# stwerner97/model-based-pde-control

Measured on AMD Instinct MI355X. Metric: KS sub-steps/sec (batched env), higher is better.
Workload: dtype f64

## Files before the change

model-based-pde-control_amd/csrc/fno.hip:

```cpp
#include <hip/hip_runtime.h>

#include <cstdio>
#include <map>
#include <mutex>
#include <utility>

#include "../../include/spectral/forward_select.h"
#include "../../include/spectral_hip.h"
#include "capi_error.h"

namespace {

typedef float f32x4 __attribute__((ext_vector_type(4)));

constexpr int C = 32;
constexpr int M = 16;
constexpr int K2 = 2 * M;
constexpr int KP = K2 + 4;
constexpr int KS = 2;
constexpr int TPB = 512;
constexpr int LAYERS = 4;

struct Weights {
    const float* lift_w;
    const float* lift_b;
    const float* wr[LAYERS];
    const float* wi[LAYERS];
    const float* pw[LAYERS];
    const float* pb[LAYERS];
    const float* p1_w;
    const float* p1_b;
    const float* p2_w;
    const float* p2_b;
};

struct Rows {
    const float* ptr;
    long stride_t, stride_b;
    __device__ const float* row(int t, int b) const { return ptr + t * stride_t + b * stride_b; }
};

struct FwdArgs {
    Weights w;
    Rows u, act;
    float* delta;
    float* out;
    float* pre;
    float* xspec;
    const float* tabg;
    int n, nb, pairs;
    int spec_pairs, spec_pair0;
    float cscale, cshift;
};

struct BwdArgs {
    Weights w;
    Rows u, act;
    const float* gdelta;
    const float* gout;
    int gout_t;
    const float* pre;
    float* gspec;
    float* rows;
    float* dbase;
    float* dact;
    const float* tabg;
    int n, nb, pairs;
    int spec_pairs, spec_pair0;
    float cscale;
};

constexpr int R_LIFT_W = 0, R_LIFT_B = 64, R_LAYER = 96, R_LAYER_SZ = 1024 + 32;
constexpr int R_P1W = R_LAYER + LAYERS * R_LAYER_SZ, R_P1B = R_P1W + 1024, R_P2W = R_P1B + 32, R_P2B = R_P2W + 32;
constexpr int ROW = ((R_P2B + 1 + 63) / 64) * 64;

__device__ __forceinline__ void gelu_parts(float x, float& cdf, float& pdf) {
    const float ax = fabsf(x);
    const float e = __expf(-0.5f * x * x);
    const float t = __frcp_rn(fmaf(0.3275911f * 0.70710678118654752f, ax, 1.0f));
    float poly = fmaf(1.061405429f, t, -1.453152027f);
    poly = fmaf(poly, t, 1.421413741f);
    poly = fmaf(poly, t, -0.284496736f);
    poly = fmaf(poly, t, 0.254829592f);
    const float erf_abs = fmaf(-poly * t, e, 1.0f);
    cdf = 0.5f * (1.0f + copysignf(erf_abs, x));
    pdf = 0.3989422804014327f * e;
}
__device__ __forceinline__ float gelu(float x) {
    float cdf, pdf;
    gelu_parts(x, cdf, pdf);
    return x * cdf;
}
__device__ __forceinline__ float gelu_grad(float x) {
    float cdf, pdf;
    gelu_parts(x, cdf, pdf);
    return fmaf(x, pdf, cdf);
}

#ifdef FNO_STAMP
__device__ unsigned long long g_stamps[256];
#define STAMP(k)                                                                      \
    do {                                                                              \
        if (blockIdx.x == 0 && threadIdx.x == 0) g_stamps[(k)] = __builtin_amdgcn_s_memtime(); \
    } while (0)
#else
#define STAMP(k) do { } while (0)
#endif

struct Lds {
    float *xs, *tb, *S, *Z, *wps, *gv, *misc;
    int NP;
    __device__ Lds(float* base, int N) {
        NP = N + 4;
        xs = base;
        tb = xs + C * NP;
        S = tb + C * NP;
        Z = S + KS * C * KP;
        wps = Z + C * KP;
        gv = wps + C * KP;
        misc = gv + N;
    }
    static size_t floats(int N) { return 2 * (size_t)C * (N + 4) + (KS + 2) * C * KP + (size_t)N + 256; }
};

__global__ void twiddle_init_kernel(float* tab, int N) {
    const int i = blockIdx.x * blockDim.x + threadIdx.x;
    if (i >= K2 * N) return;
    const int k = i / N, n = i - k * N;
    const bool is_sin = k >= M;
    const int mode = is_sin ? k - M : k;
    const int idx = (int)(((long)mode * n) % N);
    const float ang = 2.0f * (float)idx / (float)N;
    tab[i] = is_sin ? -sinpif(ang) : cospif(ang);
}
__device__ __forceinline__ void load_table(float* tab, const float* __restrict__ tabg, int N, int NP) {
    const int sh = __ffs(N) - 1;
    for (int i = threadIdx.x; i < (K2 * N) >> 2; i += blockDim.x) {
        const int e = i << 2, k = e >> sh, n = e & (N - 1);
        *reinterpret_cast<float4*>(tab + k * NP + n) = reinterpret_cast<const float4*>(tabg)[i];
    }
}

__device__ __forceinline__ void contract_n(const float* arows, const float* brows, float* S, int N, int NP) {
    const int lane = threadIdx.x & 63, wave = threadIdx.x >> 6, nwaves = blockDim.x >> 6;
    const int r = lane & 15, q = lane >> 4;
    for (int t = wave; t < 4 * KS; t += nwaves) {
        const int tile = t & 3, ks = t >> 2, rt = tile >> 1, ct = tile & 1;
        const int span = N / KS, kbeg = ks * span;
        const float* arow = arows + (16 * rt + r) * NP + kbeg;
        const float* brow = brows + (16 * ct + r) * NP + kbeg;
        f32x4 acc0 = {0.f, 0.f, 0.f, 0.f}, acc1 = {0.f, 0.f, 0.f, 0.f}, acc2 = {0.f, 0.f, 0.f, 0.f}, acc3 = {0.f, 0.f, 0.f, 0.f};
        for (int k0 = 0; k0 < span; k0 += 16) {
            const float a0 = arow[k0 + q], a1 = arow[k0 + 4 + q], a2 = arow[k0 + 8 + q], a3 = arow[k0 + 12 + q];
            const float b0 = brow[k0 + q], b1 = brow[k0 + 4 + q], b2 = brow[k0 + 8 + q], b3 = brow[k0 + 12 + q];
            acc0 = __builtin_amdgcn_mfma_f32_16x16x4f32(a0, b0, acc0, 0, 0, 0);
            acc1 = __builtin_amdgcn_mfma_f32_16x16x4f32(a1, b1, acc1, 0, 0, 0);
            acc2 = __builtin_amdgcn_mfma_f32_16x16x4f32(a2, b2, acc2, 0, 0, 0);
            acc3 = __builtin_amdgcn_mfma_f32_16x16x4f32(a3, b3, acc3, 0, 0, 0);
        }
        float* dst = S + ks * C * KP;
// ... 273 lines not shown
            const float* wrow = L.wps + (16 * rt + r) * KP;
#pragma unroll
            for (int k0 = 0; k0 < C; k0 += 4)
                acc = __builtin_amdgcn_mfma_f32_16x16x4f32(wrow[k0 + q], L.xs[(k0 + q) * NP + pos], acc, 0, 0, 0);
#pragma unroll
            for (int j = 0; j < 4; ++j) {
                const int row = 16 * rt + 4 * q + j;
                part = fmaf(L.misc[C + row], gelu(acc[j] + L.misc[row]), part);
            }
        }
        part += __shfl_xor(part, 16, 64);
        part += __shfl_xor(part, 32, 64);
        if (q == 0) {
            const float d = part + b2;
            out[pos] = fmaf(cscale, d, u[pos]) + cshift;
        }
    }
}

__device__ __forceinline__ float row_dot(const float* buf, const float* v, int N, int NP) {
    const int row = threadIdx.x >> 4, l16 = threadIdx.x & 15;
    float s = 0.0f;
    if (row < C) {
        const float* src = buf + row * NP;
        if (v) {
            for (int n = l16; n < N; n += 16) s = fmaf(src[n], v[n], s);
        } else {
            for (int n = l16; n < N; n += 16) s += src[n];
        }
    }
    s += __shfl_xor(s, 1, 64);
    s += __shfl_xor(s, 2, 64);
    s += __shfl_xor(s, 4, 64);
    s += __shfl_xor(s, 8, 64);
    return s;
}

__global__ void __launch_bounds__(TPB) fno_backward_kernel(const BwdArgs a) {
    extern __shared__ __align__(16) float lds_raw[];
    const int N = a.n;
    const Lds L(lds_raw, N);
    const int NP = L.NP;
    float* db = L.tb;
    const int p = blockIdx.x, t = p / a.nb, b = p - t * a.nb;
    const int lane = threadIdx.x & 63, wave = threadIdx.x >> 6, nwaves = blockDim.x >> 6;
    const int r = lane & 15, q = lane >> 4;
    const int sh = __ffs(N) - 1;
    const float* u = a.u.row(t, b);
    const float* act = a.act.row(t, b);
    float* grow = a.rows + (size_t)p * ROW;
    const float* pre_p = a.pre + (size_t)p * LAYERS * C * N;
    const bool has_gout = a.gout && t == a.gout_t;

    for (int n = threadIdx.x; n < N; n += blockDim.x) {
        float g = a.gdelta[(size_t)p * N + n];
        if (has_gout) g = fmaf(a.cscale, a.gout[(size_t)b * N + n], g);
        L.gv[n] = g;
    }
    {
        const float4* src = reinterpret_cast<const float4*>(pre_p + (size_t)(LAYERS - 1) * C * N);
        for (int i = threadIdx.x; i < (C * N) >> 2; i += blockDim.x) {
            const int e = i << 2, c = e >> sh, n = e & (N - 1);
            *reinterpret_cast<float4*>(L.xs + c * NP + n) = src[i];
        }
    }
    load_mat(L.wps, a.w.p1_w);
    if (threadIdx.x < C) {
        L.misc[threadIdx.x] = a.w.p1_b[threadIdx.x];
        L.misc[C + threadIdx.x] = a.w.p2_w[threadIdx.x];
    }
    __syncthreads();

    {
        float dw2[2][4] = {{0.f, 0.f, 0.f, 0.f}, {0.f, 0.f, 0.f, 0.f}};
        for (int ct = wave; ct < (N >> 4); ct += nwaves) {
            const int pos = 16 * ct + r;
            const float g = L.gv[pos];
#pragma unroll
            for (int rt = 0; rt < 2; ++rt) {
                f32x4 acc = {0.f, 0.f, 0.f, 0.f};
                const float* wrow = L.wps + (16 * rt + r) * KP;
#pragma unroll
                for (int k0 = 0; k0 < C; k0 += 4)
                    acc = __builtin_amdgcn_mfma_f32_16x16x4f32(wrow[k0 + q], L.xs[(k0 + q) * NP + pos], acc, 0, 0, 0);
#pragma unroll
                for (int j = 0; j < 4; ++j) {
                    const int row = 16 * rt + 4 * q + j;
                    const float z1 = acc[j] + L.misc[row];
                    dw2[rt][j] = fmaf(g, gelu(z1), dw2[rt][j]);
                    db[row * NP + pos] = L.misc[C + row] * g * gelu_grad(z1);
                }
            }
        }
#pragma unroll
        for (int rt = 0; rt < 2; ++rt)
#pragma unroll
            for (int j = 0; j < 4; ++j) {
                float v = dw2[rt][j];
                v += __shfl_xor(v, 1, 64);
                v += __shfl_xor(v, 2, 64);
                v += __shfl_xor(v, 4, 64);
                v += __shfl_xor(v, 8, 64);
                if (r == 0) L.Z[wave * C + 16 * rt + 4 * q + j] = v;
            }
    }
    __syncthreads();
    contract_n(db, L.xs, L.S, N, NP);
    {
        const float s = row_dot(db, nullptr, N, NP);
        if ((threadIdx.x & 15) == 0 && (threadIdx.x >> 4) < C) grow[R_P1B + (threadIdx.x >> 4)] = s;
        if (threadIdx.x < C) {
            float v = L.Z[threadIdx.x];
            for (int w = 1; w < TPB / 64; ++w) v += L.Z[w * C + threadIdx.x];
            grow[R_P2W + threadIdx.x] = v;
        }
        if (wave == 0) {
            float g = 0.0f;
            for (int n = lane; n < N; n += 64) g += L.gv[n];
#pragma unroll
            for (int m = 1; m < 64; m <<= 1) g += __shfl_xor(g, m, 64);
            if (lane == 0) grow[R_P2B] = g;
        }
    }
    __syncthreads();
    for (int i = threadIdx.x; i < C * C; i += blockDim.x) grow[R_P1W + i] = s_sum(L.S, (i >> 5) * KP + (i & 31));
    for (int ct = wave; ct < (N >> 4); ct += nwaves) {
        const int pos = 16 * ct + r;
        f32x4 acc[2];
#pragma unroll
        for (int rt = 0; rt < 2; ++rt) {
            acc[rt] = f32x4{0.f, 0.f, 0.f, 0.f};
#pragma unroll
            for (int k0 = 0; k0 < C; k0 += 4)
                acc[rt] = __builtin_amdgcn_mfma_f32_16x16x4f32(L.wps[(k0 + q) * KP + 16 * rt + r], db[(k0 + q) * NP + pos], acc[rt], 0, 0, 0);
        }
#pragma unroll
        for (int rt = 0; rt < 2; ++rt)
#pragma unroll
            for (int j = 0; j < 4; ++j) db[(16 * rt + 4 * q + j) * NP + pos] = acc[rt][j];
    }
    __syncthreads();

    const float s0 = 1.0f / (float)N, s1 = 2.0f / (float)N;
    for (int l = LAYERS - 1; l >= 0; --l) {
        if (l + 1 < LAYERS) {
            const float4* src = reinterpret_cast<const float4*>(pre_p + (size_t)l * C * N);
            for (int i = threadIdx.x; i < (C * N) >> 2; i += blockDim.x) {
                const int e = i << 2, c = e >> sh, n = e & (N - 1);
                const float4 v = src[i];
                float4* d = reinterpret_cast<float4*>(db + c * NP + n);
                float4 g = *d;
                g.x *= gelu_grad(v.x);
                g.y *= gelu_grad(v.y);
                g.z *= gelu_grad(v.z);
                g.w *= gelu_grad(v.w);
                *d = g;
            }
        }
        if (l > 0) {
            const float4* src = reinterpret_cast<const float4*>(pre_p + (size_t)(l - 1) * C * N);
            for (int i = threadIdx.x; i < (C * N) >> 2; i += blockDim.x) {
                const int e = i << 2, c = e >> sh, n = e & (N - 1);
                float4 v = src[i];
                v.x = gelu(v.x);
                v.y = gelu(v.y);
                v.z = gelu(v.z);
                v.w = gelu(v.w);
                *reinterpret_cast<float4*>(L.xs + c * NP + n) = v;
            }
        } else {
            lift_into(L.xs, u, act, a.w, N, NP);
        }
        load_mat(L.wps, a.w.pw[l]);
        __syncthreads();
        contract_n(db, L.xs, L.S, N, NP);
        {
            const float s = row_dot(db, nullptr, N, NP);
            if ((threadIdx.x & 15) == 0 && (threadIdx.x >> 4) < C) grow[R_LAYER + l * R_LAYER_SZ + 1024 + (threadIdx.x >> 4)] = s;
        }
        __syncthreads();
        for (int i = threadIdx.x; i < C * C; i += blockDim.x)
            grow[R_LAYER + l * R_LAYER_SZ + i] = s_sum(L.S, (i >> 5) * KP + (i & 31));
        load_table(L.xs, a.tabg, N, NP);
        __syncthreads();
        MixRegs mw;
        mix_load<true>(a.w.wr[l], a.w.wi[l], mw);
        contract_n(db, L.xs, L.S, N, NP);
        __syncthreads();
        for (int i = threadIdx.x; i < C * K2; i += blockDim.x) {
            const int k = i >> 5, c = i & 31, m = k & (M - 1);
            const float g = s_sum(L.S, c * KP + k) * (m == 0 ? s0 : s1);
            L.Z[c * KP + k] = g;
            a.gspec[(((size_t)l * K2 + k) * a.spec_pairs + a.spec_pair0 + p) * C + c] = g;
        }
        __syncthreads();
        mix_compute<true>(mw, L.Z, L.S, 1.0f, 1.0f);
        __syncthreads();
        for (int ct = wave; ct < (N >> 4); ct += nwaves) {
            const int pos = 16 * ct + r;
            f32x4 acc[2][2];
#pragma unroll
            for (int rt = 0; rt < 2; ++rt) {
                acc[rt][0] = f32x4{0.f, 0.f, 0.f, 0.f};
                acc[rt][1] = f32x4{0.f, 0.f, 0.f, 0.f};
                const float* zrow = L.S + (16 * rt + r) * KP;
#pragma unroll
                for (int k0 = 0; k0 < K2; k0 += 4) {
                    acc[rt][0] = __builtin_amdgcn_mfma_f32_16x16x4f32(zrow[k0 + q], L.xs[(k0 + q) * NP + pos], acc[rt][0], 0, 0, 0);
                    acc[rt][1] = __builtin_amdgcn_mfma_f32_16x16x4f32(L.wps[(k0 + q) * KP + 16 * rt + r], db[(k0 + q) * NP + pos], acc[rt][1], 0, 0, 0);
                }
            }
#pragma unroll
            for (int rt = 0; rt < 2; ++rt)
#pragma unroll
                for (int j = 0; j < 4; ++j) db[(16 * rt + 4 * q + j) * NP + pos] = acc[rt][0][j] + acc[rt][1][j];
        }
        __syncthreads();
    }

    for (int n = threadIdx.x; n < N; n += blockDim.x) {
        L.gv[n] = u[n];
        L.Z[n] = act[n];
    }
    if (threadIdx.x < C) {
        L.misc[threadIdx.x] = a.w.lift_w[2 * threadIdx.x];
        L.misc[C + threadIdx.x] = a.w.lift_w[2 * threadIdx.x + 1];
    }
    __syncthreads();
    {
        const float su = row_dot(db, L.gv, N, NP), sa = row_dot(db, L.Z, N, NP), sb = row_dot(db, nullptr, N, NP);
        if ((threadIdx.x & 15) == 0 && (threadIdx.x >> 4) < C) {
            const int c = threadIdx.x >> 4;
            grow[R_LIFT_W + 2 * c] = su;
            grow[R_LIFT_W + 2 * c + 1] = sa;
            grow[R_LIFT_B + c] = sb;
        }
    }
    if (a.dbase) {
        for (int n = threadIdx.x; n < N; n += blockDim.x) {
            float s = 0.0f;
#pragma unroll 8
            for (int c = 0; c < C; ++c) s = fmaf(L.misc[c], db[c * NP + n], s);
            if (has_gout) s += a.gout[(size_t)b * N + n];
            a.dbase[(size_t)p * N + n] = s;
        }
    }
    if (a.dact) {
        for (int n = threadIdx.x; n < N; n += blockDim.x) {
            float s = 0.0f;
#pragma unroll 8
            for (int c = 0; c < C; ++c) s = fmaf(L.misc[C + c], db[c * NP + n], s);
            a.dact[(size_t)p * N + n] = s;
        }
    }
}

__global__ void __launch_bounds__(512) fno_reduce_rows_kernel(const float* rows, int pairs, int width, float* out) {
    __shared__ float part[8][64];
    const int col = threadIdx.x & 63, grp = threadIdx.x >> 6;
    const int j = blockIdx.x * 64 + col;
    float s0 = 0.0f, s1 = 0.0f, s2 = 0.0f, s3 = 0.0f;
    if (j < width) {
        int p = grp;
        for (; p + 24 < pairs; p += 32) {
            s0 += rows[(size_t)p * width + j];
            s1 += rows[(size_t)(p + 8) * width + j];
            s2 += rows[(size_t)(p + 16) * width + j];
            s3 += rows[(size_t)(p + 24) * width + j];
        }
        for (; p < pairs; p += 8) s0 += rows[(size_t)p * width + j];
    }
    part[grp][col] = (s0 + s1) + (s2 + s3);
    __syncthreads();
    if (grp == 0 && j < width) {
        float v = part[0][col];
#pragma unroll
        for (int g = 1; g < 8; ++g) v += part[g][col];
        out[j] = v;
    }
}

struct WgradOut {
    float* dwr[LAYERS];
    float* dwi[LAYERS];
};

constexpr int WG_KS = 4;
__global__ void __launch_bounds__(256 * WG_KS) fno_spec_wgrad_kernel(const float* xspec, const float* gspec, int pairs, const WgradOut dst) {
    __shared__ float part[WG_KS][4][2][256];
    const int l = blockIdx.x / M, m = blockIdx.x % M;
    const int lane = threadIdx.x & 63, wave = threadIdx.x >> 6;
    const int tile = wave & 3, ks = wave >> 2;
    const int r = lane & 15, q = lane >> 4;
    const int rt = tile >> 1, ct = tile & 1;
    const size_t plane = (size_t)pairs * C;
    const float* xr = xspec + ((size_t)l * K2 + m) * plane;
    const float* xi = xspec + ((size_t)l * K2 + M + m) * plane;
    const float* gr = gspec + ((size_t)l * K2 + m) * plane;
    const float* gi = gspec + ((size_t)l * K2 + M + m) * plane;
    f32x4 rr = {0.f, 0.f, 0.f, 0.f}, ii = {0.f, 0.f, 0.f, 0.f}, ir = {0.f, 0.f, 0.f, 0.f}, ri = {0.f, 0.f, 0.f, 0.f};
    for (int p0 = 4 * ks; p0 < pairs; p0 += 4 * WG_KS) {
        const int pp = p0 + q;
        const bool ok = pp < pairs;
        const size_t row = (size_t)(ok ? pp : 0) * C;
        const float axr = ok ? xr[row + 16 * rt + r] : 0.f, axi = ok ? xi[row + 16 * rt + r] : 0.f;
        const float bgr = ok ? gr[row + 16 * ct + r] : 0.f, bgi = ok ? gi[row + 16 * ct + r] : 0.f;
// ... 150 lines not shown
    if (int rc = check(who, n, nb, nb, width, modes, layers)) return rc;
    SelectArgs k = {};
    for (int m = 0; m < a->members; ++m) {
        k.w[m] = weights_of(&a->w[m]);
        k.cscale[m] = a->cscale[m];
        k.cshift[m] = a->cshift[m];
    }
    k.chosen = a->chosen;
    k.step = a->step;
    k.u = a->u;
    k.act = a->act;
    k.out = a->out;
    k.members = a->members;
    k.T = a->T;
    k.n = n;
    k.nb = nb;
    int trc = 0;
    k.tabg = twiddle_table(who, n, (hipStream_t)stream, &trc);
    if (!k.tabg) return trc;
    return launch(fno_forward_select_kernel, who, stream, nb, n, k);
}

int fno_backward(void* stream, const fno_weights* w, int width, int modes, int layers, int n, int nb, int pairs, const float* u,
                 long u_stride_t, long u_stride_b, const float* act, long a_stride_t, long a_stride_b, float cscale,
                 const float* gdelta, const float* gout, int gout_t, const float* pre, float* gspec, int spec_pairs, int spec_pair0,
                 float* rows, float* dbase, float* dact) {
    if (!complete(w) || !u || !act || !gdelta || !pre || !gspec || !rows) return fail(-1, "fno_backward: bad argument");
    if (spec_pair0 < 0 || spec_pair0 + pairs > spec_pairs) return fail(-1, "fno_backward: spectra window out of range");
    if (int rc = check("fno_backward", n, nb, pairs, width, modes, layers)) return rc;
    BwdArgs a;
    a.w = weights_of(w);
    a.u = Rows{u, u_stride_t, u_stride_b};
    a.act = Rows{act, a_stride_t, a_stride_b};
    a.gdelta = gdelta;
    a.gout = gout;
    a.gout_t = gout_t;
    a.pre = pre;
    a.gspec = gspec;
    a.spec_pairs = spec_pairs;
    a.spec_pair0 = spec_pair0;
    a.rows = rows;
    a.dbase = dbase;
    a.dact = dact;
    int trc = 0;
    a.tabg = twiddle_table("fno_backward", n, (hipStream_t)stream, &trc);
    if (!a.tabg) return trc;
    a.n = n;
    a.nb = nb;
    a.pairs = pairs;
    a.cscale = cscale;
    return launch(fno_backward_kernel, "fno_backward", stream, pairs, n, a);
}

int fno_reduce_rows(void* stream, const float* rows, int pairs, float* out) {
    if (!rows || !out || pairs <= 0) return fail(-1, "fno_reduce_rows: bad argument");
    hipLaunchKernelGGL(fno_reduce_rows_kernel, dim3((ROW + 63) / 64), dim3(512), 0, (hipStream_t)stream, rows, pairs, ROW, out);
    return launch_status(-2, "fno_reduce_rows");
}

int fno_spec_wgrad(void* stream, const float* xspec, const float* gspec, int pairs, float* const* dwr, float* const* dwi) {
    if (!xspec || !gspec || !dwr || !dwi || pairs <= 0) return fail(-1, "fno_spec_wgrad: bad argument");
    WgradOut dst;
    for (int l = 0; l < LAYERS; ++l) {
        if (!dwr[l] || !dwi[l]) return fail(-1, "fno_spec_wgrad: NULL output");
        dst.dwr[l] = dwr[l];
        dst.dwi[l] = dwi[l];
    }
    hipLaunchKernelGGL(fno_spec_wgrad_kernel, dim3(LAYERS * M), dim3(256 * WG_KS), 0, (hipStream_t)stream, xspec, gspec, pairs, dst);
    return launch_status(-2, "fno_spec_wgrad");
}

const char* fno_last_error(void) { return g_err; }

#ifdef FNO_STAMP
int fno_read_stamps(unsigned long long* host, int n) {
    return hipMemcpyFromSymbol(host, HIP_SYMBOL(g_stamps), sizeof(unsigned long long) * (n < 256 ? n : 256)) == hipSuccess ? 0 : -2;
}
#endif

}
```

model-based-pde-control_amd/pdecontrol/surrogates/fno_hip.py:

```python
import ctypes

import torch

import hipbind
from pdecontrol.surrogates import spectral

_p, _i, _l, _f = ctypes.c_void_p, ctypes.c_int, ctypes.c_long, ctypes.c_float
WIDTH, MODES, LAYERS = 32, 16, 4


class FnoWeights(ctypes.Structure):
    _fields_ = [("lift_w", _p), ("lift_b", _p), ("spec_wr", _p * 4), ("spec_wi", _p * 4), ("pw_w", _p * 4), ("pw_b", _p * 4),
                ("p1_w", _p), ("p1_b", _p), ("p2_w", _p), ("p2_b", _p)]


_WP = ctypes.POINTER(FnoWeights)
SYMBOLS = (
    ("fno_forward", _i, [_p, _WP, _i, _i, _i, _i, _i, _i, _p, _l, _l, _p, _l, _l, _f, _f, _p, _p, _p, _p, _i, _i]),
    ("fno_backward", _i, [_p, _WP, _i, _i, _i, _i, _i, _i, _p, _l, _l, _p, _l, _l, _f, _p, _p, _i, _p, _p, _i, _i, _p, _p, _p]),
    ("fno_row_width", _i, []),
    ("fno_reduce_rows", _i, [_p, _p, _i, _p]),
    ("fno_spec_wgrad", _i, [_p, _p, _p, _i, _p * 4, _p * 4]),
    ("fno_last_error", ctypes.c_char_p, []),
)
MAX_MEMBERS = 8


class FnoSelectArgs(ctypes.Structure):
    _fields_ = [("w", _WP), ("cscale", ctypes.POINTER(_f)), ("cshift", ctypes.POINTER(_f)), ("members", _i), ("chosen", _p),
                ("step", _p), ("T", _i), ("u", _p), ("act", _p), ("out", _p)]


SELECT_SYMBOLS = (
    ("fno_forward_select", _i, [_p, _i, _i, _i, _i, _i, ctypes.POINTER(FnoSelectArgs)]),
)
_lib = None


class FnoHipError(RuntimeError):
    pass


def load():
    global _lib
    if _lib is None:
        _lib = hipbind.type_symbols(spectral.load(), SYMBOLS + SELECT_SYMBOLS)
    return _lib


_check = hipbind.checker(FnoHipError, "libspectral_hip (fno)", "fno_last_error", lambda: load())
_stream, _ptr = hipbind.stream, hipbind.ptr


def parameters_of(model):
    ps = [model.lift.weight, model.lift.bias]
    for spec, pw in zip(model.spectral, model.pointwise):
        ps += [spec.weight_real, spec.weight_imag, pw.weight, pw.bias]
    ps += [model.project[0].weight, model.project[0].bias, model.project[2].weight, model.project[2].bias]
    return ps


def supported(model, n):
    try:
        return (len(model.spectral) == LAYERS and model.lift.weight.shape == (WIDTH, 2)
                and all(s.in_channels == WIDTH and s.out_channels == WIDTH and s.modes == MODES for s in model.spectral)
                and isinstance(model.activation, torch.nn.GELU) and getattr(model.activation, "approximate", "none") == "none"
                and 64 <= n <= 512 and (n & (n - 1)) == 0 and model.lift.weight.dtype == torch.float32)
    except AttributeError:
        return False


def _weights_struct(params):
    w = FnoWeights()
    ps = [p.detach() if p.is_contiguous() else p.detach().contiguous() for p in params]
    w.lift_w, w.lift_b = ps[0].data_ptr(), ps[1].data_ptr()
    for layer in range(LAYERS):
        wr, wi, pw, pb = ps[2 + 4 * layer: 6 + 4 * layer]
        w.spec_wr[layer], w.spec_wi[layer], w.pw_w[layer], w.pw_b[layer] = wr.data_ptr(), wi.data_ptr(), pw.data_ptr(), pb.data_ptr()
    base = 2 + 4 * LAYERS
    w.p1_w, w.p1_b, w.p2_w, w.p2_b = (ps[base + k].data_ptr() for k in range(4))
    return w, ps


def affine_of(dscaling):
    from pdecontrol.surrogates import hipops
    try:
        mul, add = hipops._dscale_constants(dscaling)
    except hipops.SurrogateHipError:
        return None
    return float(mul), float(add)


def world_supported(surrogate, n):
    from pdecontrol.architectures.fno import FNOAutoRegSurrogate
    return (isinstance(surrogate, FNOAutoRegSurrogate) and supported(surrogate.model, int(n))
            and affine_of(surrogate.dscaling) is not None)


def select_args(surrogates, chosen, step, T, u, act, out):
    assert 1 <= len(surrogates) <= MAX_MEMBERS
    M = len(surrogates)
    ws, keep, cscale, cshift = (FnoWeights * M)(), [], (_f * M)(), (_f * M)()
    for m, sur in enumerate(surrogates):
        w, ps = _weights_struct(parameters_of(sur.model))
        ws[m] = w
        keep.append(ps)
        scale, shift = affine_of(sur.dscaling)
        cscale[m], cshift[m] = float(sur.delta) * scale, float(sur.delta) * shift
    a = FnoSelectArgs(ws, cscale, cshift, M, *(None if t is None else t.data_ptr() for t in (chosen, step)), int(T),
                      u.data_ptr(), act.data_ptr(), out.data_ptr())
    a._keep = (ws, cscale, cshift, keep)
    return a


def forward_select(stream, n, nb, args):
    _check(load().fno_forward_select(stream, WIDTH, MODES, LAYERS, int(n), int(nb), ctypes.byref(args)))


def _launch_groups(n_given, K):
    return [(0, n_given)] + [(k, 1) for k in range(n_given, K)]


def _forward_launches(lib, w, states, acts, n_given, cscale, cshift, deltas, outputs, pre, xspec, spec_pairs, pair0):
    B, K, N = acts.shape[0], acts.shape[1], acts.shape[-1]
    st = _stream()
    ast, asb = acts.stride(1), acts.stride(0)
    for k0, cnt in _launch_groups(n_given, K):
        if k0 < n_given:
            u_ptr, ust, usb = states.data_ptr(), states.stride(1), states.stride(0)
        else:
            u_ptr, ust, usb = outputs[k0 - 1].data_ptr(), 0, outputs.stride(1)
        _check(lib.fno_forward(st, ctypes.byref(w), WIDTH, MODES, LAYERS, N, B, cnt * B, ctypes.c_void_p(u_ptr), ust, usb,
                               ctypes.c_void_p(acts.data_ptr() + 4 * k0 * ast), ast, asb, cscale, cshift,
                               _ptr(deltas[k0]), _ptr(outputs[k0]), _ptr(None if pre is None else pre[k0 * B:]), _ptr(xspec),
                               spec_pairs, pair0 + k0 * B))


def _backward_launches(lib, w, states, acts, outputs, pre, n_given, cscale, g_deltas, gspec, spec_pairs, pair0, rows, gouts,
                       g_outputs=None, dstates=None, dacts=None):
    B, K, N = acts.shape[0], acts.shape[1], acts.shape[-1]
    st = _stream()
    ast, asb = acts.stride(1), acts.stride(0)
    gout = None
    for k0, cnt in reversed(_launch_groups(n_given, K)):
        free = k0 >= n_given
        if free:
            u_ptr, ust, usb = outputs[k0 - 1].data_ptr(), 0, outputs.stride(1)
            if g_outputs is not None:
                gout = g_outputs[k0] if gout is None else gout.add_(g_outputs[k0])
        else:
            u_ptr, ust, usb = states.data_ptr(), states.stride(1), states.stride(0)
        new_gout = gouts[k0 - n_given] if free else dstates
        _check(lib.fno_backward(st, ctypes.byref(w), WIDTH, MODES, LAYERS, N, B, cnt * B, ctypes.c_void_p(u_ptr), ust, usb,
                                ctypes.c_void_p(acts.data_ptr() + 4 * k0 * ast), ast, asb, cscale,
                                _ptr(g_deltas[k0]), _ptr(gout), (0 if free else n_given - 1), _ptr(pre[k0 * B:]), _ptr(gspec),
                                spec_pairs, pair0 + k0 * B, _ptr(rows[k0 * B:]), _ptr(new_gout),
                                _ptr(None if dacts is None else dacts[k0])))
        gout = new_gout


def _parameter_grads(lib, rows, xspec, gspec, pairs, needs):
    dev = rows.device
    st = _stream()
    width = rows.shape[1]
    flat = torch.empty(width, device=dev, dtype=torch.float32)
    _check(lib.fno_reduce_rows(st, _ptr(rows), pairs, _ptr(flat)))
    dwr = [torch.empty((WIDTH, WIDTH, MODES), device=dev, dtype=torch.float32) for _ in range(LAYERS)]
    dwi = [torch.empty((WIDTH, WIDTH, MODES), device=dev, dtype=torch.float32) for _ in range(LAYERS)]
    _check(lib.fno_spec_wgrad(st, _ptr(xspec), _ptr(gspec), pairs, (_p * 4)(*[t.data_ptr() for t in dwr]),
                              (_p * 4)(*[t.data_ptr() for t in dwi])))
    grads = [flat[0:64].view(32, 2), flat[64:96]]
    off = 96
    for layer in range(LAYERS):
        grads += [dwr[layer], dwi[layer], flat[off:off + 1024].view(32, 32), flat[off + 1024:off + 1056]]
        off += 1056
    grads += [flat[off:off + 1024].view(32, 32), flat[off + 1024:off + 1056], flat[off + 1056:off + 1088].view(1, 32),
              flat[off + 1088:off + 1089]]
    return [g if need else None for g, need in zip(grads, needs)]


class _FNORolloutFn(torch.autograd.Function):

    @staticmethod
    def forward(ctx, states, acts, n_given, cscale, cshift, *params):
        lib = load()
        states, acts = states.contiguous(), acts.contiguous()
        B, K, N = acts.shape[0], acts.shape[1], acts.shape[-1]
        n_given = min(int(n_given), K)
        dev = states.device
        need = any(ctx.needs_input_grad[:2]) or any(ctx.needs_input_grad[5:])
        w, keep = _weights_struct(params)
        deltas = torch.empty((K, B, N), device=dev, dtype=torch.float32)
        outputs = torch.empty((K, B, N), device=dev, dtype=torch.float32)
        pre = torch.empty((K * B, LAYERS, WIDTH, N), device=dev, dtype=torch.float32) if need else None
        xspec = torch.empty((LAYERS, 2 * MODES, K * B, WIDTH), device=dev, dtype=torch.float32) if need else None
        _forward_launches(lib, w, states, acts, n_given, cscale, cshift, deltas, outputs, pre, xspec, K * B, 0)
        ctx.need = need
        if need:
            ctx.save_for_backward(states, acts, outputs, pre, xspec, *params)
            ctx.meta = (B, K, N, n_given, float(cscale))
        ctx.set_materialize_grads(False)
        del keep
        return deltas, outputs

    @staticmethod
    def backward(ctx, g_deltas, g_outputs):
        if not ctx.need or (g_deltas is None and g_outputs is None):
            return (None,) * len(ctx.needs_input_grad)
        lib = load()
        B, K, N, n_given, cscale = ctx.meta
        saved = ctx.saved_tensors
# ... 30 lines not shown
class _FNOTBPTTFn(torch.autograd.Function):

    @staticmethod
    def forward(ctx, states, actions, tau, tbtt, cscale, cshift, *params):
        lib = load()
        states, actions = states.contiguous(), actions.contiguous()
        B, T, N = actions.shape[0], actions.shape[1], actions.shape[-1]
        dev = states.device
        need = any(ctx.needs_input_grad[6:])
        w, keep = _weights_struct(params)
        deltas = torch.empty((T, B, N), device=dev, dtype=torch.float32)
        outputs = torch.empty((T, B, N), device=dev, dtype=torch.float32)
        pre = torch.empty((T * B, LAYERS, WIDTH, N), device=dev, dtype=torch.float32) if need else None
        xspec = torch.empty((LAYERS, 2 * MODES, T * B, WIDTH), device=dev, dtype=torch.float32) if need else None
        chunks = []
        for k0 in range(0, T, tbtt):
            K = min(tbtt, T - k0)
            if k0 == 0:
                seed, n_given = states[:, :min(tau, K)], min(tau, K)
            else:
                seed, n_given = outputs[k0 - 1].view(B, 1, 1, N), 1
            chunks.append((k0, K, n_given, seed))
            _forward_launches(lib, w, seed, actions[:, k0:k0 + K], n_given, cscale, cshift, deltas[k0:], outputs[k0:],
                              None if pre is None else pre[k0 * B:], xspec, T * B, k0 * B)
        ctx.need = need
        if need:
            ctx.save_for_backward(states, actions, outputs, pre, xspec, *params)
            ctx.meta = (B, T, N, float(cscale), [(k0, K, ng) for k0, K, ng, _ in chunks], int(tau))
        ctx.set_materialize_grads(False)
        del keep
        return deltas, outputs

    @staticmethod
    def backward(ctx, g_deltas, g_outputs):
        if not ctx.need or (g_deltas is None and g_outputs is None):
            return (None,) * len(ctx.needs_input_grad)
        from pdecontrol.surrogates import hipops
        lib = load()
        B, T, N, cscale, chunks, tau = ctx.meta
        saved = ctx.saved_tensors
        states, actions, outputs, pre, xspec = saved[:5]
        params = saved[5:]
        dev = states.device
        w, keep = _weights_struct(params)
        g_deltas = torch.zeros_like(outputs) if g_deltas is None else g_deltas.contiguous()
        if g_outputs is not None:
            g_outputs = g_outputs.contiguous()
            g_deltas = g_deltas.clone()
            for k0, _, ng in chunks:
                g_deltas[k0:k0 + ng].add_(g_outputs[k0:k0 + ng], alpha=cscale)
        rows = torch.empty((T * B, lib.fno_row_width()), device=dev, dtype=torch.float32)
        gspec = torch.empty((LAYERS, 2 * MODES, T * B, WIDTH), device=dev, dtype=torch.float32)
        gouts = [[torch.empty((B, N), device=dev, dtype=torch.float32) for _ in range(K - ng)] for _, K, ng in chunks]
        streams = hipops.pooled_streams(dev, max(len(chunks) - 1, 0), "side")
        forks = []
        for c, (k0, K, ng) in enumerate(chunks):
            seed = states[:, :ng] if k0 == 0 else outputs[k0 - 1].view(B, 1, 1, N)
            args = (lib, w, seed, actions[:, k0:k0 + K], outputs[k0:], pre[k0 * B:], ng, cscale, g_deltas[k0:], gspec, T * B,
                    k0 * B, rows[k0 * B:], gouts[c], None if g_outputs is None else g_outputs[k0:])
            if c + 1 < len(chunks):
                fork = hipops._Fork(streams[c])
                with fork:
                    _backward_launches(*args)
                forks.append(fork)
            else:
                _backward_launches(*args)
        for fork in forks:
            fork.join()
        out = _parameter_grads(lib, rows, xspec, gspec, T * B, ctx.needs_input_grad[6:])
        del keep
        return (None, None, None, None, None, None, *out)


def tbptt(surrogate, states, actions, tau, tbtt, grid):
    from pdecontrol.surrogates.surrogate import action_and_target_indices, take_steps
    model = surrogate.model
    if states.dtype != torch.float32 or states.dim() != 4 or states.shape[2] != 1 or actions.shape != states.shape:
        return None
    if states.requires_grad or actions.requires_grad:
        return None
    n, T = states.shape[-1], actions.shape[1]
    if not supported(model, n):
        return None
    aff = affine_of(surrogate.dscaling)
    if aff is None:
        return None
    gidx = []
    for k0 in range(0, T, tbtt):
        K = min(tbtt, T - k0)
        aidx, tidx = action_and_target_indices(*grid(K), surrogate.delta)
        aidx, tidx = aidx.tolist(), tidx.tolist()
        if tidx != list(range(K)) or len(aidx) < K or min(aidx[:K]) < 0 or max(aidx[:K]) >= K:
            return None
        gidx += [k0 + j for j in aidx[:K]]
    acts = actions if gidx == list(range(T)) else take_steps(actions, gidx)
    scale, shift = aff
    d, o = _FNOTBPTTFn.apply(states, acts, int(tau), int(tbtt), float(surrogate.delta) * scale, float(surrogate.delta) * shift,
                             *parameters_of(model))
    return o.transpose(0, 1).unsqueeze(2), d.transpose(0, 1).unsqueeze(2), d.unsqueeze(2)


def rollout(model, states, actions, n_given, delta, dscaling):
    if states.dtype != torch.float32 or states.dim() != 4 or states.shape[2] != 1 or actions.shape[2] != 1:
        return None
    n = states.shape[-1]
    if not supported(model, n):
        return None
    aff = affine_of(dscaling)
    if aff is None:
        return None
    scale, shift = aff
    d, o = _FNORolloutFn.apply(states, actions, int(n_given), float(delta) * scale, float(delta) * shift, *parameters_of(model))
    return d.transpose(0, 1).unsqueeze(2), o.transpose(0, 1).unsqueeze(2)
```

Measured before the change: 1.378 billion.

## Split FNO backward into chain and weight-gradient kernels overlapped across streams

```diff
diff --git a/include/spectral/backward_split.h b/include/spectral/backward_split.h
--- /dev/null
+++ b/include/spectral/backward_split.h
@@ -0,0 +1,25 @@
+#ifndef SPECTRAL_BACKWARD_SPLIT_H
+#define SPECTRAL_BACKWARD_SPLIT_H
+
+#include "../spectral_hip.h"
+
+#ifdef __cplusplus
+extern "C" {
+#endif
+
+#define FNO_DPRE_SLOTS 5
+
+int fno_backward_chain(void* stream, const fno_weights* w, int width, int modes, int layers, int n, int nb, int pairs, const float* u,
+                       long u_stride_t, long u_stride_b, const float* act, long a_stride_t, long a_stride_b, float cscale,
+                       const float* gdelta, const float* gout, int gout_t, const float* pre, float* gspec, int spec_pairs,
+                       int spec_pair0, float* rows, float* dbase, float* dact, float* dpre);
+
+int fno_backward_wgrad(void* stream, const fno_weights* w, int width, int modes, int layers, int n, int nb, int pairs, const float* u,
+                       long u_stride_t, long u_stride_b, const float* act, long a_stride_t, long a_stride_b, const float* pre,
+                       const float* dpre, float* rows);
+
+#ifdef __cplusplus
+}
+#endif
+
+#endif
diff --git a/model-based-pde-control_amd/csrc/fno.hip b/model-based-pde-control_amd/csrc/fno.hip
--- a/model-based-pde-control_amd/csrc/fno.hip
+++ b/model-based-pde-control_amd/csrc/fno.hip
@@ -1,10 +1,12 @@
 #include <hip/hip_runtime.h>
 
+#include <climits>
 #include <cstdio>
 #include <map>
 #include <mutex>
 #include <utility>
 
+#include "../../include/spectral/backward_split.h"
 #include "../../include/spectral/forward_select.h"
 #include "../../include/spectral_hip.h"
 #include "capi_error.h"
@@ -106,6 +108,7 @@
 #else
 #define STAMP(k) do { } while (0)
 #endif
+[[maybe_unused]] constexpr int BS = 32, BS_LAYER = 40, CS = 64;
 
 struct Lds {
     float *xs, *tb, *S, *Z, *wps, *gv, *misc;
@@ -485,6 +488,7 @@
     const float* pre_p = a.pre + (size_t)p * LAYERS * C * N;
     const bool has_gout = a.gout && t == a.gout_t;
 
+    STAMP(BS + 0);
     for (int n = threadIdx.x; n < N; n += blockDim.x) {
         float g = a.gdelta[(size_t)p * N + n];
         if (has_gout) g = fmaf(a.cscale, a.gout[(size_t)b * N + n], g);
@@ -538,6 +542,7 @@
             }
     }
     __syncthreads();
+    STAMP(BS + 1);
     contract_n(db, L.xs, L.S, N, NP);
     {
         const float s = row_dot(db, nullptr, N, NP);
@@ -557,6 +562,7 @@
     }
     __syncthreads();
     for (int i = threadIdx.x; i < C * C; i += blockDim.x) grow[R_P1W + i] = s_sum(L.S, (i >> 5) * KP + (i & 31));
+    STAMP(BS + 2);
     for (int ct = wave; ct < (N >> 4); ct += nwaves) {
         const int pos = 16 * ct + r;
         f32x4 acc[2];
@@ -573,9 +579,11 @@
             for (int j = 0; j < 4; ++j) db[(16 * rt + 4 * q + j) * NP + pos] = acc[rt][j];
     }
     __syncthreads();
+    STAMP(BS + 3);
 
     const float s0 = 1.0f / (float)N, s1 = 2.0f / (float)N;
     for (int l = LAYERS - 1; l >= 0; --l) {
+        STAMP(BS_LAYER + 8 * l);
         if (l + 1 < LAYERS) {
             const float4* src = reinterpret_cast<const float4*>(pre_p + (size_t)l * C * N);
             for (int i = threadIdx.x; i < (C * N) >> 2; i += blockDim.x) {
@@ -590,6 +598,7 @@
                 *d = g;
             }
         }
+        STAMP(BS_LAYER + 8 * l + 1);
         if (l > 0) {
             const float4* src = reinterpret_cast<const float4*>(pre_p + (size_t)(l - 1) * C * N);
             for (int i = threadIdx.x; i < (C * N) >> 2; i += blockDim.x) {
@@ -606,6 +615,7 @@
         }
         load_mat(L.wps, a.w.pw[l]);
         __syncthreads();
+        STAMP(BS_LAYER + 8 * l + 2);
         contract_n(db, L.xs, L.S, N, NP);
         {
             const float s = row_dot(db, nullptr, N, NP);
@@ -614,12 +624,15 @@
         __syncthreads();
         for (int i = threadIdx.x; i < C * C; i += blockDim.x)
             grow[R_LAYER + l * R_LAYER_SZ + i] = s_sum(L.S, (i >> 5) * KP + (i & 31));
+        STAMP(BS_LAYER + 8 * l + 3);
         load_table(L.xs, a.tabg, N, NP);
         __syncthreads();
+        STAMP(BS_LAYER + 8 * l + 4);
         MixRegs mw;
         mix_load<true>(a.w.wr[l], a.w.wi[l], mw);
         contract_n(db, L.xs, L.S, N, NP);
         __syncthreads();
+        STAMP(BS_LAYER + 8 * l + 5);
         for (int i = threadIdx.x; i < C * K2; i += blockDim.x) {
             const int k = i >> 5, c = i & 31, m = k & (M - 1);
             const float g = s_sum(L.S, c * KP + k) * (m == 0 ? s0 : s1);
@@ -629,6 +642,7 @@
         __syncthreads();
         mix_compute<true>(mw, L.Z, L.S, 1.0f, 1.0f);
         __syncthreads();
+        STAMP(BS_LAYER + 8 * l + 6);
         for (int ct = wave; ct < (N >> 4); ct += nwaves) {
             const int pos = 16 * ct + r;
             f32x4 acc[2][2];
@@ -649,8 +663,10 @@
                 for (int j = 0; j < 4; ++j) db[(16 * rt + 4 * q + j) * NP + pos] = acc[rt][0][j] + acc[rt][1][j];
         }
         __syncthreads();
-    }
-
+        STAMP(BS_LAYER + 8 * l + 7);
+    }
+
+    STAMP(BS + 4);
     for (int n = threadIdx.x; n < N; n += blockDim.x) {
         L.gv[n] = u[n];
         L.Z[n] = act[n];
@@ -685,6 +701,298 @@
             for (int c = 0; c < C; ++c) s = fmaf(L.misc[C + c], db[c * NP + n], s);
             a.dact[(size_t)p * N + n] = s;
         }
+    }
+    STAMP(BS + 5);
+}
+
+constexpr int DPRE_SLOTS = FNO_DPRE_SLOTS;
+
+struct ChainArgs {
+    BwdArgs a;
+    float* dpre;
+};
+
+struct WgradArgs {
+    Weights w;
+    Rows u, act;
+    const float* pre;
+    const float* dpre;
+    float* rows;
+    int n, nb, pairs;
+};
+
+__device__ __forceinline__ void store_slot(float* __restrict__ dst, const float* db, int N, int NP, int sh) {
+    for (int i = threadIdx.x; i < (C * N) >> 2; i += blockDim.x) {
+        const int e = i << 2, c = e >> sh, n = e & (N - 1);
+        reinterpret_cast<float4*>(dst)[i] = *reinterpret_cast<const float4*>(db + c * NP + n);
+    }
+}
+
+__global__ void __launch_bounds__(TPB) fno_backward_chain_kernel(const ChainArgs ca) {
+    extern __shared__ __align__(16) float lds_raw[];
+    const BwdArgs& a = ca.a;
+    const int N = a.n;
+    const Lds L(lds_raw, N);
+    const int NP = L.NP;
+    float* db = L.tb;
+    const int p = blockIdx.x, t = p / a.nb, b = p - t * a.nb;
+    const int lane = threadIdx.x & 63, wave = threadIdx.x >> 6, nwaves = blockDim.x >> 6;
+    const int r = lane & 15, q = lane >> 4;
+    const int sh = __ffs(N) - 1;
+    const float* u = a.u.row(t, b);
+    const float* act = a.act.row(t, b);
+    float* grow = a.rows + (size_t)p * ROW;
+    const float* pre_p = a.pre + (size_t)p * LAYERS * C * N;
+    float* dpre_p = ca.dpre + (size_t)p * DPRE_SLOTS * C * N;
+    const bool has_gout = a.gout && t == a.gout_t;
+
+    STAMP(CS + BS + 0);
+    for (int n = threadIdx.x; n < N; n += blockDim.x) {
+        float g = a.gdelta[(size_t)p * N + n];
+        if (has_gout) g = fmaf(a.cscale, a.gout[(size_t)b * N + n], g);
+        L.gv[n] = g;
+    }
+    {
+        const float4* src = reinterpret_cast<const float4*>(pre_p + (size_t)(LAYERS - 1) * C * N);
+        for (int i = threadIdx.x; i < (C * N) >> 2; i += blockDim.x) {
+            const int e = i << 2, c = e >> sh, n = e & (N - 1);
+            *reinterpret_cast<float4*>(L.xs + c * NP + n) = src[i];
+        }
+    }
+    load_mat(L.wps, a.w.p1_w);
+    if (threadIdx.x < C) {
+        L.misc[threadIdx.x] = a.w.p1_b[threadIdx.x];
+        L.misc[C + threadIdx.x] = a.w.p2_w[threadIdx.x];
+    }
+    __syncthreads();
+
+    {
+        float dw2[2][4] = {{0.f, 0.f, 0.f, 0.f}, {0.f, 0.f, 0.f, 0.f}};
+        for (int ct = wave; ct < (N >> 4); ct += nwaves) {
+            const int pos = 16 * ct + r;
+            const float g = L.gv[pos];
+#pragma unroll
+            for (int rt = 0; rt < 2; ++rt) {
+                f32x4 acc = {0.f, 0.f, 0.f, 0.f};
+                const float* wrow = L.wps + (16 * rt + r) * KP;
+#pragma unroll
+                for (int k0 = 0; k0 < C; k0 += 4)
+                    acc = __builtin_amdgcn_mfma_f32_16x16x4f32(wrow[k0 + q], L.xs[(k0 + q) * NP + pos], acc, 0, 0, 0);
+#pragma unroll
+                for (int j = 0; j < 4; ++j) {
+                    const int row = 16 * rt + 4 * q + j;
+                    const float z1 = acc[j] + L.misc[row];
+                    dw2[rt][j] = fmaf(g, gelu(z1), dw2[rt][j]);
+                    db[row * NP + pos] = L.misc[C + row] * g * gelu_grad(z1);
+                }
+            }
+        }
+#pragma unroll
+        for (int rt = 0; rt < 2; ++rt)
+#pragma unroll
+            for (int j = 0; j < 4; ++j) {
+                float v = dw2[rt][j];
+                v += __shfl_xor(v, 1, 64);
+                v += __shfl_xor(v, 2, 64);
+                v += __shfl_xor(v, 4, 64);
+                v += __shfl_xor(v, 8, 64);
+                if (r == 0) L.Z[wave * C + 16 * rt + 4 * q + j] = v;
+            }
+    }
+    __syncthreads();
+    STAMP(CS + BS + 1);
+    store_slot(dpre_p + (size_t)LAYERS * C * N, db, N, NP, sh);
+    load_table(L.xs, a.tabg, N, NP);
+    {
+        if (threadIdx.x < C) {
+            float v = L.Z[threadIdx.x];
+            for (int w = 1; w < TPB / 64; ++w) v += L.Z[w * C + threadIdx.x];
+            grow[R_P2W + threadIdx.x] = v;
+        }
+        if (wave == 0) {
+            float g = 0.0f;
+            for (int n = lane; n < N; n += 64) g += L.gv[n];
+#pragma unroll
+            for (int m = 1; m < 64; m <<= 1) g += __shfl_xor(g, m, 64);
+            if (lane == 0) grow[R_P2B] = g;
+        }
+    }
+    __syncthreads();
+    STAMP(CS + BS + 2);
+    for (int ct = wave; ct < (N >> 4); ct += nwaves) {
+        const int pos = 16 * ct + r;
+        f32x4 acc[2];
+#pragma unroll
+        for (int rt = 0; rt < 2; ++rt) {
+            acc[rt] = f32x4{0.f, 0.f, 0.f, 0.f};
+#pragma unroll
+            for (int k0 = 0; k0 < C; k0 += 4)
+                acc[rt] = __builtin_amdgcn_mfma_f32_16x16x4f32(L.wps[(k0 + q) * KP + 16 * rt + r], db[(k0 + q) * NP + pos], acc[rt], 0, 0, 0);
+        }
+#pragma unroll
+        for (int rt = 0; rt < 2; ++rt)
+#pragma unroll
+            for (int j = 0; j < 4; ++j) db[(16 * rt + 4 * q + j) * NP + pos] = acc[rt][j];
+    }
+    __syncthreads();
+    STAMP(CS + BS + 3);
+
+    const float s0 = 1.0f / (float)N, s1 = 2.0f / (float)N;
+    for (int l = LAYERS - 1; l >= 0; --l) {
+        STAMP(CS + BS_LAYER + 8 * l);
+        float* slot = dpre_p + (size_t)l * C * N;
+        if (l + 1 < LAYERS) {
+            const float4* src = reinterpret_cast<const float4*>(pre_p + (size_t)l * C * N);
+            for (int i = threadIdx.x; i < (C * N) >> 2; i += blockDim.x) {
+                const int e = i << 2, c = e >> sh, n = e & (N - 1);
+                const float4 v = src[i];
+                float4* d = reinterpret_cast<float4*>(db + c * NP + n);
+                float4 g = *d;
+                g.x *= gelu_grad(v.x);
+                g.y *= gelu_grad(v.y);
+                g.z *= gelu_grad(v.z);
+                g.w *= gelu_grad(v.w);
+                *d = g;
+                reinterpret_cast<float4*>(slot)[i] = g;
+            }
+        } else {
+            store_slot(slot, db, N, NP, sh);
+        }
+        STAMP(CS + BS_LAYER + 8 * l + 1);
+        load_mat(L.wps, a.w.pw[l]);
+        __syncthreads();
+        STAMP(CS + BS_LAYER + 8 * l + 2);
+        STAMP(CS + BS_LAYER + 8 * l + 3);
+        STAMP(CS + BS_LAYER + 8 * l + 4);
+        MixRegs mw;
+        mix_load<true>(a.w.wr[l], a.w.wi[l], mw);
+        contract_n(db, L.xs, L.S, N, NP);
+        __syncthreads();
+        STAMP(CS + BS_LAYER + 8 * l + 5);
+        for (int i = threadIdx.x; i < C * K2; i += blockDim.x) {
+            const int k = i >> 5, c = i & 31, m = k & (M - 1);
+            const float g = s_sum(L.S, c * KP + k) * (m == 0 ? s0 : s1);
+            L.Z[c * KP + k] = g;
+            a.gspec[(((size_t)l * K2 + k) * a.spec_pairs + a.spec_pair0 + p) * C + c] = g;
+        }
+        __syncthreads();
+        mix_compute<true>(mw, L.Z, L.S, 1.0f, 1.0f);
+        __syncthreads();
+        STAMP(CS + BS_LAYER + 8 * l + 6);
+        for (int ct = wave; ct < (N >> 4); ct += nwaves) {
+            const int pos = 16 * ct + r;
+            f32x4 acc[2][2];
+#pragma unroll
+            for (int rt = 0; rt < 2; ++rt) {
+                acc[rt][0] = f32x4{0.f, 0.f, 0.f, 0.f};
+                acc[rt][1] = f32x4{0.f, 0.f, 0.f, 0.f};
+                const float* zrow = L.S + (16 * rt + r) * KP;
+#pragma unroll
+                for (int k0 = 0; k0 < K2; k0 += 4) {
+                    acc[rt][0] = __builtin_amdgcn_mfma_f32_16x16x4f32(zrow[k0 + q], L.xs[(k0 + q) * NP + pos], acc[rt][0], 0, 0, 0);
+                    acc[rt][1] = __builtin_amdgcn_mfma_f32_16x16x4f32(L.wps[(k0 + q) * KP + 16 * rt + r], db[(k0 + q) * NP + pos], acc[rt][1], 0, 0, 0);
+                }
+            }
+#pragma unroll
+            for (int rt = 0; rt < 2; ++rt)
+#pragma unroll
+                for (int j = 0; j < 4; ++j) db[(16 * rt + 4 * q + j) * NP + pos] = acc[rt][0][j] + acc[rt][1][j];
+        }
+        __syncthreads();
+        STAMP(CS + BS_LAYER + 8 * l + 7);
+    }
+
+    STAMP(CS + BS + 4);
+    for (int n = threadIdx.x; n < N; n += blockDim.x) {
+        L.gv[n] = u[n];
+        L.Z[n] = act[n];
+    }
+    if (threadIdx.x < C) {
+        L.misc[threadIdx.x] = a.w.lift_w[2 * threadIdx.x];
+        L.misc[C + threadIdx.x] = a.w.lift_w[2 * threadIdx.x + 1];
+    }
+    __syncthreads();
+    {
+        const float su = row_dot(db, L.gv, N, NP), sa = row_dot(db, L.Z, N, NP), sb = row_dot(db, nullptr, N, NP);
+        if ((threadIdx.x & 15) == 0 && (threadIdx.x >> 4) < C) {
+            const int c = threadIdx.x >> 4;
+            grow[R_LIFT_W + 2 * c] = su;
+            grow[R_LIFT_W + 2 * c + 1] = sa;
+            grow[R_LIFT_B + c] = sb;
+        }
+    }
+    if (a.dbase) {
+        for (int n = threadIdx.x; n < N; n += blockDim.x) {
+            float s = 0.0f;
+#pragma unroll 8
+            for (int c = 0; c < C; ++c) s = fmaf(L.misc[c], db[c * NP + n], s);
+            if (has_gout) s += a.gout[(size_t)b * N + n];
+            a.dbase[(size_t)p * N + n] = s;
+        }
+    }
+    if (a.dact) {
+        for (int n = threadIdx.x; n < N; n += blockDim.x) {
+            float s = 0.0f;
+#pragma unroll 8
+            for (int c = 0; c < C; ++c) s = fmaf(L.misc[C + c], db[c * NP + n], s);
+            a.dact[(size_t)p * N + n] = s;
+        }
+    }
+    STAMP(CS + BS + 5);
+}
+
+#ifndef FNO_WGRAD_GRID
+#define FNO_WGRAD_GRID INT_MAX
+#endif
+__global__ void __launch_bounds__(TPB) fno_backward_wgrad_kernel(const WgradArgs a) {
+    extern __shared__ __align__(16) float lds_raw[];
+    const int N = a.n;
+    const Lds L(lds_raw, N);
+    const int NP = L.NP;
+    float* db = L.tb;
+    const int sh = __ffs(N) - 1;
+    for (int item = blockIdx.x; item < a.pairs * DPRE_SLOTS; item += gridDim.x) {
+        const int p = item / DPRE_SLOTS, slot = item - p * DPRE_SLOTS;
+        const int t = p / a.nb, b = p - t * a.nb;
+        float* grow = a.rows + (size_t)p * ROW;
+        const float* pre_p = a.pre + (size_t)p * LAYERS * C * N;
+        {
+            const float4* src = reinterpret_cast<const float4*>(a.dpre + ((size_t)p * DPRE_SLOTS + slot) * C * N);
+            for (int i = threadIdx.x; i < (C * N) >> 2; i += blockDim.x) {
+                const int e = i << 2, c = e >> sh, n = e & (N - 1);
+                *reinterpret_cast<float4*>(db + c * NP + n) = src[i];
+            }
+        }
+        if (slot == LAYERS) {
+            const float4* src = reinterpret_cast<const float4*>(pre_p + (size_t)(LAYERS - 1) * C * N);
+            for (int i = threadIdx.x; i < (C * N) >> 2; i += blockDim.x) {
+                const int e = i << 2, c = e >> sh, n = e & (N - 1);
+                *reinterpret_cast<float4*>(L.xs + c * NP + n) = src[i];
+            }
+        } else if (slot > 0) {
+            const float4* src = reinterpret_cast<const float4*>(pre_p + (size_t)(slot - 1) * C * N);
+            for (int i = threadIdx.x; i < (C * N) >> 2; i += blockDim.x) {
+                const int e = i << 2, c = e >> sh, n = e & (N - 1);
+                float4 v = src[i];
+                v.x = gelu(v.x);
+                v.y = gelu(v.y);
+                v.z = gelu(v.z);
+                v.w = gelu(v.w);
+                *reinterpret_cast<float4*>(L.xs + c * NP + n) = v;
+            }
+        } else {
+            lift_into(L.xs, a.u.row(t, b), a.act.row(t, b), a.w, N, NP);
+        }
+        __syncthreads();
+        const int wcol = slot == LAYERS ? R_P1W : R_LAYER + slot * R_LAYER_SZ;
+        contract_n(db, L.xs, L.S, N, NP);
+        {
+            const float s = row_dot(db, nullptr, N, NP);
+            if ((threadIdx.x & 15) == 0 && (threadIdx.x >> 4) < C) grow[wcol + 1024 + (threadIdx.x >> 4)] = s;
+        }
+        __syncthreads();
+        for (int i = threadIdx.x; i < C * C; i += blockDim.x) grow[wcol + i] = s_sum(L.S, (i >> 5) * KP + (i & 31));
+        __syncthreads();
     }
 }
 
@@ -941,6 +1249,63 @@
     return launch(fno_backward_kernel, "fno_backward", stream, pairs, n, a);
 }
 
+int fno_backward_chain(void* stream, const fno_weights* w, int width, int modes, int layers, int n, int nb, int pairs, const float* u,
+                       long u_stride_t, long u_stride_b, const float* act, long a_stride_t, long a_stride_b, float cscale,
+                       const float* gdelta, const float* gout, int gout_t, const float* pre, float* gspec, int spec_pairs,
+                       int spec_pair0, float* rows, float* dbase, float* dact, float* dpre) {
+    const char* who = "fno_backward_chain";
+    if (!complete(w) || !u || !act || !gdelta || !pre || !gspec) return fail(-1, "%s: bad argument", who);
+    if (!rows || !dpre) return fail(-1, "%s: NULL rows or dpre", who);
+    if (spec_pair0 < 0 || spec_pair0 + pairs > spec_pairs) return fail(-1, "%s: spectra window out of range", who);
+    if (int rc = check(who, n, nb, pairs, width, modes, layers)) return rc;
+    ChainArgs c;
+    BwdArgs& a = c.a;
+    a.w = weights_of(w);
+    a.u = Rows{u, u_stride_t, u_stride_b};
+    a.act = Rows{act, a_stride_t, a_stride_b};
+    a.gdelta = gdelta;
+    a.gout = gout;
+    a.gout_t = gout_t;
+    a.pre = pre;
+    a.gspec = gspec;
+    a.spec_pairs = spec_pairs;
+    a.spec_pair0 = spec_pair0;
+    a.rows = rows;
+    a.dbase = dbase;
+    a.dact = dact;
+    int trc = 0;
+    a.tabg = twiddle_table(who, n, (hipStream_t)stream, &trc);
+    if (!a.tabg) return trc;
+    a.n = n;
+    a.nb = nb;
+    a.pairs = pairs;
+    a.cscale = cscale;
+    c.dpre = dpre;
+    return launch(fno_backward_chain_kernel, who, stream, pairs, n, c);
+}
+
+int fno_backward_wgrad(void* stream, const fno_weights* w, int width, int modes, int layers, int n, int nb, int pairs, const float* u,
+                       long u_stride_t, long u_stride_b, const float* act, long a_stride_t, long a_stride_b, const float* pre,
+                       const float* dpre, float* rows) {
+    const char* who = "fno_backward_wgrad";
+    if (!complete(w) || !u || !act || !pre) return fail(-1, "%s: bad argument", who);
+    if (!rows || !dpre) return fail(-1, "%s: NULL rows or dpre", who);
+    if (int rc = check(who, n, nb, pairs, width, modes, layers)) return rc;
+    if (pairs > INT_MAX / DPRE_SLOTS) return fail(-1, "%s: %d pairs are more than one launch takes", who, pairs);
+    WgradArgs a;
+    a.w = weights_of(w);
+    a.u = Rows{u, u_stride_t, u_stride_b};
+    a.act = Rows{act, a_stride_t, a_stride_b};
+    a.pre = pre;
+    a.dpre = dpre;
+    a.rows = rows;
+    a.n = n;
+    a.nb = nb;
+    a.pairs = pairs;
+    const int items = pairs * DPRE_SLOTS;
+    return launch(fno_backward_wgrad_kernel, who, stream, items < FNO_WGRAD_GRID ? items : FNO_WGRAD_GRID, n, a);
+}
+
 int fno_reduce_rows(void* stream, const float* rows, int pairs, float* out) {
     if (!rows || !out || pairs <= 0) return fail(-1, "fno_reduce_rows: bad argument");
     hipLaunchKernelGGL(fno_reduce_rows_kernel, dim3((ROW + 63) / 64), dim3(512), 0, (hipStream_t)stream, rows, pairs, ROW, out);
diff --git a/model-based-pde-control_amd/pdecontrol/surrogates/fno_hip.py b/model-based-pde-control_amd/pdecontrol/surrogates/fno_hip.py
--- a/model-based-pde-control_amd/pdecontrol/surrogates/fno_hip.py
+++ b/model-based-pde-control_amd/pdecontrol/surrogates/fno_hip.py
@@ -1,4 +1,5 @@
 import ctypes
+import os
 
 import torch
 
@@ -34,7 +35,17 @@
 SELECT_SYMBOLS = (
     ("fno_forward_select", _i, [_p, _i, _i, _i, _i, _i, ctypes.POINTER(FnoSelectArgs)]),
 )
+SPLIT_SYMBOLS = (
+    ("fno_backward_chain", _i, [_p, _WP, _i, _i, _i, _i, _i, _i, _p, _l, _l, _p, _l, _l, _f, _p, _p, _i, _p, _p, _i, _i, _p, _p, _p,
+                                _p]),
+    ("fno_backward_wgrad", _i, [_p, _WP, _i, _i, _i, _i, _i, _i, _p, _l, _l, _p, _l, _l, _p, _p, _p]),
+)
+DPRE_SLOTS = 5
 _lib = None
+
+
+def split_backward():
+    return os.environ.get("PDECONTROL_FNO_SPLIT_BWD", "1") != "0"
 
 
 class FnoHipError(RuntimeError):
@@ -44,7 +55,7 @@
 def load():
     global _lib
     if _lib is None:
-        _lib = hipbind.type_symbols(spectral.load(), SYMBOLS + SELECT_SYMBOLS)
+        _lib = hipbind.type_symbols(spectral.load(), SYMBOLS + SELECT_SYMBOLS + SPLIT_SYMBOLS)
     return _lib
 
 
@@ -136,14 +147,26 @@
                                spec_pairs, pair0 + k0 * B))
 
 
-def _backward_launches(lib, w, states, acts, outputs, pre, n_given, cscale, g_deltas, gspec, spec_pairs, pair0, rows, gouts,
-                       g_outputs=None, dstates=None, dacts=None):
+def _backward_launches(*args, **kwargs):
+    for _ in _backward_steps(*args, **kwargs):
+        pass
+
+
+def _backward_steps(lib, w, states, acts, outputs, pre, n_given, cscale, g_deltas, gspec, spec_pairs, pair0, rows, gouts,
+                    g_outputs=None, dstates=None, dacts=None, split=None):
     B, K, N = acts.shape[0], acts.shape[1], acts.shape[-1]
-    st = _stream()
     ast, asb = acts.stride(1), acts.stride(0)
     gout = None
+    pending = None
+
+    def wgrad(event, wargs):
+        dpre, wstream = split
+        if event is not None:
+            wstream.wait_event(event)
+        _check(lib.fno_backward_wgrad(ctypes.c_void_p(wstream.cuda_stream), *wargs))
     for k0, cnt in reversed(_launch_groups(n_given, K)):
         free = k0 >= n_given
+        st = _stream()
         if free:
             u_ptr, ust, usb = outputs[k0 - 1].data_ptr(), 0, outputs.stride(1)
             if g_outputs is not None:
@@ -151,12 +174,27 @@
         else:
             u_ptr, ust, usb = states.data_ptr(), states.stride(1), states.stride(0)
         new_gout = gouts[k0 - n_given] if free else dstates
-        _check(lib.fno_backward(st, ctypes.byref(w), WIDTH, MODES, LAYERS, N, B, cnt * B, ctypes.c_void_p(u_ptr), ust, usb,
-                                ctypes.c_void_p(acts.data_ptr() + 4 * k0 * ast), ast, asb, cscale,
-                                _ptr(g_deltas[k0]), _ptr(gout), (0 if free else n_given - 1), _ptr(pre[k0 * B:]), _ptr(gspec),
-                                spec_pairs, pair0 + k0 * B, _ptr(rows[k0 * B:]), _ptr(new_gout),
-                                _ptr(None if dacts is None else dacts[k0])))
+        rows_of = (ctypes.byref(w), WIDTH, MODES, LAYERS, N, B, cnt * B, ctypes.c_void_p(u_ptr), ust, usb,
+                   ctypes.c_void_p(acts.data_ptr() + 4 * k0 * ast), ast, asb)
+        chain = (cscale, _ptr(g_deltas[k0]), _ptr(gout), (0 if free else n_given - 1), _ptr(pre[k0 * B:]), _ptr(gspec),
+                 spec_pairs, pair0 + k0 * B, _ptr(rows[k0 * B:]), _ptr(new_gout), _ptr(None if dacts is None else dacts[k0]))
+        if split is None:
+            _check(lib.fno_backward(st, *rows_of, *chain))
+        else:
+            dpre, wstream = split
+            _check(lib.fno_backward_chain(st, *rows_of, *chain, _ptr(dpre[k0 * B:])))
+            event = None
+            if wstream.cuda_stream != st.value:
+                event = torch.cuda.Event()
+                event.record(torch.cuda.current_stream(acts.device))
+            if pending is not None:
+                wgrad(*pending)
+            pending = (event, (*rows_of, _ptr(pre[k0 * B:]), _ptr(dpre[k0 * B:]), _ptr(rows[k0 * B:])))
         gout = new_gout
+        if k0 > 0:
+            yield
+    if pending is not None:
+        wgrad(*pending)
 
 
 def _parameter_grads(lib, rows, xspec, gspec, pairs, needs):
@@ -293,19 +331,43 @@
         rows = torch.empty((T * B, lib.fno_row_width()), device=dev, dtype=torch.float32)
         gspec = torch.empty((LAYERS, 2 * MODES, T * B, WIDTH), device=dev, dtype=torch.float32)
         gouts = [[torch.empty((B, N), device=dev, dtype=torch.float32) for _ in range(K - ng)] for _, K, ng in chunks]
-        streams = hipops.pooled_streams(dev, max(len(chunks) - 1, 0), "side")
-        forks = []
-        for c, (k0, K, ng) in enumerate(chunks):
+        split = split_backward() and not torch.cuda.is_current_stream_capturing()
+        dpre = torch.empty((T * B, DPRE_SLOTS, WIDTH, N), device=dev, dtype=torch.float32) if split else None
+        streams = hipops.pooled_streams(dev, len(chunks) if split else max(len(chunks) - 1, 0), "side")
+        main = torch.cuda.current_stream(dev)
+        forks, walks = [], []
+        fork_point = None
+        if split:
+            fork_point = torch.cuda.Event()
+            fork_point.record(main)
+        order = sorted(range(len(chunks)), key=lambda c: -len(_launch_groups(chunks[c][2], chunks[c][1]))) if split \
+            else range(len(chunks))
+        for c in order:
+            k0, K, ng = chunks[c]
             seed = states[:, :ng] if k0 == 0 else outputs[k0 - 1].view(B, 1, 1, N)
             args = (lib, w, seed, actions[:, k0:k0 + K], outputs[k0:], pre[k0 * B:], ng, cscale, g_deltas[k0:], gspec, T * B,
                     k0 * B, rows[k0 * B:], gouts[c], None if g_outputs is None else g_outputs[k0:])
-            if c + 1 < len(chunks):
+            if split:
+                fork = hipops._Fork(streams[c], after=fork_point)
+                with fork:
+                    walk = _backward_steps(*args, split=(dpre[k0 * B:], main))
+                    if next(walk, walks) is not walks:
+                        walks.append((fork.stream, walk))
+                forks.append(fork)
+            elif c + 1 < len(chunks):
                 fork = hipops._Fork(streams[c])
                 with fork:
                     _backward_launches(*args)
                 forks.append(fork)
             else:
                 _backward_launches(*args)
+        while walks:
+            live = []
+            for stream, walk in walks:
+                with torch.cuda.stream(stream):
+                    if next(walk, walks) is not walks:
+                        live.append((stream, walk))
+            walks = live
         for fork in forks:
             fork.join()
         out = _parameter_grads(lib, rows, xspec, gspec, T * B, ctx.needs_input_grad[6:])
```

Result: no change. 1.378 billion (median of 4 runs) (+0.0%).
